# rubychen0611/image-analogies-python

Measured on AMD Instinct MI355X. Metric: B' pixels/sec (brute-force match, 5-level pyramid) + MFMA util @1/2/4/8 GPU, higher is better.
Workload: dtype f16 rotated split (R16 MFMA screen: 3 principal components as f16 pairs, 52 as f16, f32 accumulate) + f64 (rotation, exact rescore, pyramids); 1 GPU; c4: A/A' 2048x2048 x B 1024x1024, 5-level, DB sharded, brute force; levels_cap=5, jobs_per_gpu=1, streams_per_gpu=1, jobs_per_launch=1, parallelism=single

## Files before the change

image-analogies-python_amd/_ia.py:

```python
import ctypes
import os
import re
import sys

import numpy as np
import torch

_HERE = os.path.dirname(os.path.abspath(__file__))
LIB_PATH = os.environ.get('IA_LIB_PATH') or os.path.join(_HERE, 'libia.so')
HEADER = os.path.join(os.path.dirname(_HERE), 'include', 'ia.h')

IA_D = 55
IA_DP = 56

_dp = ctypes.c_void_p


class IaSrcLevel(ctypes.Structure):
    _fields_ = [('A_sm', _dp), ('A_lg', _dp), ('Ap_sm', _dp), ('Ap_lg', _dp),
                ('A_hs', ctypes.c_int), ('A_ws', ctypes.c_int), ('Ah', ctypes.c_int),
                ('Aw', ctypes.c_int), ('nAp', ctypes.c_int)]


class IaLsh(ctypes.Structure):
# ... 141 lines not shown
    'ia_diag_screen3': (ctypes.c_int, [_dp, ctypes.c_long, _dp, ctypes.c_int, _dp, _dp, _dp]),
    'ia_diag_xwave_trace': (ctypes.c_int, [_dp]),
    'ia_diag_set_db_build_form': (ctypes.c_int, [ctypes.c_int]),
    'ia_diag_set_pyr_form': (ctypes.c_int, [ctypes.c_int, ctypes.c_int]),
    'ia_diag_qp_rows': (ctypes.c_int, [ctypes.c_int]),
    'ia_diag_query_rows16': (ctypes.c_int, [_dp, ctypes.c_int, _dp, _dp, _dp, _dp, _dp, _dp]),
    'ia_diag_screen16': (ctypes.c_int, [_dp, ctypes.c_long, _dp, ctypes.c_int, _dp, _dp]),
    'ia_diag_stage_map': (ctypes.c_int, [ctypes.c_long, ctypes.c_long, ctypes.c_int, ctypes.c_int,
                                         ctypes.POINTER(ctypes.c_int)]),
    'ia_diag_screen16_rows': (ctypes.c_int, [ctypes.POINTER(IaSrcLevel), ctypes.c_long, ctypes.c_long,
                                             _dp, _dp, ctypes.c_int, _dp, _dp]),
    'ia_diag_screen16_image': (ctypes.c_int, [ctypes.POINTER(IaSrcLevel), ctypes.c_long,
                                              ctypes.c_long, _dp, _dp, ctypes.c_int, _dp, _dp]),
    'ia_diag_peer_stress': (ctypes.c_int, [_dp, ctypes.c_int, ctypes.c_int,
                                           ctypes.POINTER(ctypes.c_int), _dp]),
    'ia_diag_peer_trace': (ctypes.c_int, [_dp, _dp]),
    'ia_diag_screen16r': (ctypes.c_int, [ctypes.POINTER(IaSrcLevel), ctypes.c_long, ctypes.c_long, _dp, _dp,
                                         _dp, _dp, _dp, ctypes.c_int, _dp, _dp, _dp, _dp, _dp]),
    'ia_diag_screen16k': (ctypes.c_int, [ctypes.POINTER(IaSrcLevel), ctypes.c_long, ctypes.c_long, _dp, _dp,
                                         _dp, _dp, _dp, ctypes.c_int, _dp, _dp, _dp, _dp, _dp]),
    'ia_diag_set_compact_min_rows': (ctypes.c_long, [ctypes.c_long]),
    'ia_diag_wave_compact': (ctypes.c_int, [ctypes.c_int, ctypes.c_int]),
    'ia_diag_compact_waves': (ctypes.c_long, []),
    'ia_diag_wave_rows': (ctypes.c_int, [ctypes.c_int] * 5 + [ctypes.POINTER(ctypes.c_int)]),
    'ia_diag_pipe_schedule': (ctypes.c_int, [ctypes.POINTER(ctypes.c_int)] * 3 + [ctypes.c_int] * 3 +
                              [ctypes.POINTER(ctypes.c_int), ctypes.c_int]),
    'ia_diag_db3_askip': (ctypes.c_int, [_dp, ctypes.c_long, _dp]),
    'ia_diag_screen3r': (ctypes.c_int, [_dp, _dp, _dp, ctypes.c_long, _dp, ctypes.c_int, _dp, _dp, _dp]),
    'ia_diag_synth_level_shards': (ctypes.c_int, [ctypes.POINTER(IaSynthArgs),
                                                  ctypes.POINTER(IaShardDb), ctypes.c_int, _dp]),
}

_lib = None


def declared_symbols(header=None):
    inc = os.path.dirname(HEADER)
    if header == 'all':
        paths = [os.path.join(inc, f) for f in sorted(os.listdir(inc)) if f.endswith('.h')]
    else:
        paths = [header or HEADER]
    names = set()
    for p in paths:
        src = re.sub(r'/\*.*?\*/', '', open(p).read(), flags=re.S)
        names.update(re.findall(r'\b(ia_[a-z0-9_]+)\s*\(', src))
    return sorted(names)
# ... 269 lines not shown
```

image-analogies-python_amd/csrc/ia_internal.h:

```cpp
#pragma once
#include "ia_common.h"

#include <atomic>

namespace ia {

int rot_check_orthonormal(const float *rot, int n, int ld, hipStream_t st, const char *who);
int db_check_amax(const float *amax, hipStream_t st, const char *who);

#ifndef IA_DB_TARGET_CHUNKS
#define IA_DB_TARGET_CHUNKS 512
#endif
constexpr long DB_TARGET_CHUNKS = IA_DB_TARGET_CHUNKS;
extern thread_local long g_db_chunk_target;
constexpr int DB_CHUNK_MAX = 8192;
constexpr int DB_SEG_MAX = 512;

static inline int db_chunk_rows(long nrows) {
    const long target = g_db_chunk_target;
    const long want = (nrows + target * 128 - 1) / (target * 128);
    long tpw = 1;
    while (tpw < want && tpw < DB_CHUNK_MAX / 128) tpw <<= 1;
    return (int)(128 * tpw);
}
// ... 176 lines not shown
    gptr<const float> qp;
    gptr<const double> nq;
    gptr<const float> amax;
    gptr<const double> center;
    gptr<double> q64n;
    gptr<float> qpn;
    gptr<double> nqn;
    gptr<_Float16> q16n;
    ImgPair B, Bp;
    int H, M, y_lo_n, M_n;
    gptr<unsigned long long> dbox;
    gptr<unsigned int> tickets;
    gptr<unsigned int> err;
    gptr<unsigned long long> stats;
    FinishArgs f;
    gptr<const XJob> jobs;
    gptr<unsigned long long> trace;
    gptr<const float> rot;
    gptr<const unsigned char> askc;
    int rk;
    gptr<const unsigned char> restc;
    gptr<const float> rmax;
    gptr<const _Float16> q16;
};
constexpr int XW_TRACE_N = 17, XW_TRACE_PX = 512, XW_TRACE_T = 4096;
constexpr int XW_ROWS = 0, XW_IMG = 1, XW_STRIP = 2;
bool xstrip_applies(const DbSrc &src);
int launch_xwave(const XArgs &a, int nblocks, int form, hipStream_t st, int njobs = 1);

constexpr int STATS_SLOTS = 64, STATS_LINE = 8;
constexpr size_t STATS_BYTES = (size_t)STATS_SLOTS * STATS_LINE * sizeof(unsigned long long);
__device__ __forceinline__ unsigned long long *stats_slot(unsigned long long *s, int q) {
    return s + (q & (STATS_SLOTS - 1)) * STATS_LINE;
}

constexpr size_t MATCH_HEAD = 256;
static inline float *match_segmin(void *scratch) {
    return reinterpret_cast<float *>(reinterpret_cast<char *>(scratch) + MATCH_HEAD);
}
int exact_stage_mode();

int launch_query_wave(const ImgPair &B, const ImgPair &Bp, int t, int y_lo, int M,
                      const double *center, double *q64, float *qp, double *nq,
                      const float *amax, _Float16 *q16, hipStream_t st, const float *rot = nullptr);
int launch_screen16r(const void *dbr, long nrows, const StageMap &sm, const _Float16 *q16, int M,
                     float *segmin, hipStream_t st, const XJob *jobs = nullptr, int njobs = 1, int parity = 0,
                     bool compact = false);
long compact_min_rows();
int launch_db_amax(const IaSrcLevel *src, const DbSrc &d, const double *center, float *amax,
                   double *part, hipStream_t st);
int launch_query_rows(const double *qin, int M, const double *center, float *qp, double *nq,
                      const float *amax, _Float16 *q16, hipStream_t st);
int launch_screen16(const void *db, const ImgDb *img, long nrows, const StageMap &sm,
                    const _Float16 *q16, int M, float *segmin, hipStream_t st,
                    const XJob *jobs = nullptr, int njobs = 1, int parity = 0, bool sharded = false);
size_t match_scratch_bytes(int qrows, long nrows);
int launch_match(const DbSrc &src, long row0, long nrows, const void *db, const void *dbi,
                 const float *qp, const _Float16 *q16, int M, const double *q64, const double *nq,
                 const float *amax, void *scratch, Best *best, unsigned long long *stats,
                 hipStream_t st,
                 hipEvent_t ev0 = nullptr, hipEvent_t ev1 = nullptr,
                 const FinishArgs *fin = nullptr);
int launch_lsh_match(const IaLsh *lsh, const DbSrc &src, long row0, long nrows, int M,
                     const double *q64, const double *center, Best *best,
                     unsigned long long *stats, hipStream_t st);

}
```

image-analogies-python_amd/csrc/ia_synth.hip:

```cpp
#include "ia_finish.h"
#include "ia_split16.h"
#include "ia_rot16.h"
#include "ia_pipe.h"
#include "../../include/ia_diag.h"

#include <cstdio>
#include <cstdlib>
#include <mutex>
#include <vector>

#include <rccl/rccl.h>

namespace ia {

__device__ unsigned int g_sched_err;

__global__ __launch_bounds__(64) void k_err_sticky(const unsigned int *__restrict__ ctl,
                                                   const XJob *__restrict__ jt, int K) {
    for (int k = threadIdx.x; k < K; k += 64) {
        const unsigned int e = jt ? jt[k].ctl[2] : ctl[2];
        if (e) g_sched_err = 1u;
    }
}

// ... 98 lines not shown
    const double d_app = wv == 0 ? app_wdist(src, app, f, qs, lane) : 0.0;
    __syncthreads();
    if (wv == 0) finish_apply(src, app, m, f, cs, d_app, lane);
}

struct SynthWs {
    double *q64;
    float *qp;
    _Float16 *q16;
    double *nq;
    void *scratch;
    Best *best_local;
    ShardRec *rec_local;
    ShardRec *rec_all;
    CohSel *coh;
    unsigned long long *stats;
    double *q64b;
    float *qpb;
    _Float16 *q16b;
    double *nqb;
    unsigned long long *dbox;
    unsigned int *ctl;
    XJob *jtab;
};
constexpr int XW_CTL_ERR = 2;

static size_t carve(SynthWs *ws, char *base, int H, int W, long nrows, int nranks) {
    const int Mmax = wave_max_queries(H, W);
    const int qr = qrows_alloc(Mmax);
    size_t off = 0;
    auto take = [&](size_t bytes) { size_t o = off; off += align_up(bytes, 256); return base ? base + o : nullptr; };
    SynthWs w;
    w.q64 = (double *)take((size_t)Mmax * IA_DP * sizeof(double));
    w.qp = (float *)take((size_t)qr * IA_DP * sizeof(float));
    w.q16 = (_Float16 *)take((size_t)qr * Q16_ROW * 16);
    w.nq = (double *)take((size_t)qr * sizeof(double));
    w.scratch = take(match_scratch_bytes(qr, nrows));
    w.best_local = (Best *)take((size_t)Mmax * sizeof(Best));
    w.rec_local = (ShardRec *)take((size_t)Mmax * sizeof(ShardRec));
    w.rec_all = (ShardRec *)take((size_t)Mmax * nranks * sizeof(ShardRec));
    w.coh = (CohSel *)take((size_t)Mmax * sizeof(CohSel));
    w.stats = (unsigned long long *)take(STATS_BYTES);
    w.q64b = (double *)take((size_t)Mmax * IA_DP * sizeof(double));
    w.qpb = (float *)take((size_t)qr * IA_DP * sizeof(float));
    w.q16b = (_Float16 *)take((size_t)qr * Q16_ROW * 16);
    w.nqb = (double *)take((size_t)qr * sizeof(double));
    w.dbox = (unsigned long long *)take((size_t)H * 2 * sizeof(unsigned long long));
    w.ctl = (unsigned int *)take(256);
    w.jtab = (XJob *)take((size_t)IA_BATCH_MAX * sizeof(XJob));
    if (ws) *ws = w;
    return off;
}

struct GraphKeeper {
    hipStream_t cap = nullptr;
    hipGraphExec_t exec = nullptr;
    hipEvent_t done = nullptr;
    hipError_t retire() {
        if (!exec) return hipSuccess;
        hipError_t e = hipEventSynchronize(done);
        if (e == hipSuccess) e = hipGraphExecDestroy(exec);
        exec = nullptr;
        return e;
    }
    hipError_t hold(hipGraphExec_t x, hipStream_t st) {
        exec = x;
        if (!done) {
            hipError_t e = hipEventCreateWithFlags(&done, hipEventDisableTiming);
            if (e != hipSuccess) return e;
        }
        return hipEventRecord(done, st);
    }
// ... 40 lines not shown
        IA_HIP(hipHostMalloc(&p, STATS_BYTES, hipHostMallocDefault));
        g_prof->pinned.push_back(reinterpret_cast<unsigned long long *>(p));
    }
    *hstats = g_prof->pinned[g_prof->pinned_next++];
    return IA_OK;
}

static hipEvent_t prof_event(size_t i) {
    std::lock_guard<std::mutex> l(g_prof->mu);
    return g_prof->ev[i];
}

static void prof_push(const ProfRec &r) {
    std::lock_guard<std::mutex> l(g_prof->mu);
    g_prof->recs.push_back(r);
}

static std::atomic<int> g_graph_mode{env_int("IA_GRAPH", 0)};
static int graph_mode() { return g_graph_mode.load(std::memory_order_relaxed); }

static std::atomic<long> g_compact_min_rows{1L << 22};
long compact_min_rows() { return g_compact_min_rows.load(std::memory_order_relaxed); }
static std::atomic<long> g_compact_waves{0};

int xwave_attributes(int form, bool rot, hipFuncAttributes *at);
int screen16_attributes(bool img, hipFuncAttributes *at);
int screen_resources_r16(hipFuncAttributes *at);
int comm_allgather(void *comm, const void *send, void *recv, size_t bytes, hipStream_t st);
int comm_nranks(void *comm);
PeerView comm_peer_wave(void *comm);
int comm_peer_mcap(void *comm);

static int shard_tail() {
    static const int v = env_int("IA_SHARD_TAIL", 0);
    return v;
}

static std::atomic<int> g_xwave{env_int("IA_XWAVE", 2)};
static int xwave_on() { return g_xwave.load(std::memory_order_relaxed); }

static unsigned long long *g_xw_trace = nullptr;
static unsigned long long *xw_trace(int tag) {
    static const int want = env_int("IA_XW_TRACE", -1);
    if (want < 0 || tag != want) return nullptr;
    if (!g_xw_trace) {
        const size_t n = (size_t)XW_TRACE_T * XW_TRACE_PX * XW_TRACE_N * sizeof(unsigned long long);
// ... 53 lines not shown
        IA_HIP(hipMemsetAsync(ws.qp, 0, (size_t)qrows_alloc(Mmax) * IA_DP * sizeof(float), st));
        IA_HIP(hipMemsetAsync(ws.q16, 0, (size_t)qrows_alloc(Mmax) * Q16_ROW * 16, st));
        IA_HIP(hipMemsetAsync(ws.stats, 0, STATS_BYTES, st));
        IA_HIP(hipMemsetAsync(ws.scratch, 0, 256, st));
        src = make_dbsrc(a->src);
        B = ImgPair{a->B_sm, a->B_lg, a->B_hs, a->B_ws, H, W};
        Bp = ImgPair{a->Bp_sm, a->Bp_lg, a->B_hs, a->B_ws, H, W};
        prof = !member && (a->flags & IA_SYNTH_PROF) && prof_active();
        timed = prof;
        if (prof && (rc = prof_reserve(3 * (size_t)nw, &ev0, &hstats))) return rc;
        fused = !a->comm && !a->lsh && !sim;
        peer = a->comm && comm_peer_mcap(a->comm) > 0;
        IA_ARG(!peer || comm_peer_mcap(a->comm) >= Mmax,
               "ia_synth_level: the peer exchange's box holds fewer queries than a wave");
        IA_ARG(!peer || a->N_total < (1L << 32),
               "ia_synth_level: the peer exchange carries 32-bit rows (N_total >= 2^32)");
        xw = xwave_on() && !a->lsh && !sim && (!a->comm || peer) && exact_stage_mode() != 1;
        r16 = xw && a->dbr && a->rot;
        IA_HIP(hipMemsetAsync(ws.ctl, 0, 256, st));
        if (xw) {
            IA_HIP(hipMemsetAsync(ws.qpb, 0, (size_t)qrows_alloc(Mmax) * IA_DP * sizeof(float), st));
            IA_HIP(hipMemsetAsync(ws.q16b, 0, (size_t)qrows_alloc(Mmax) * Q16_ROW * 16, st));
            IA_HIP(hipMemsetAsync(ws.dbox, 0, (size_t)H * 2 * sizeof(unsigned long long), st));
        }
        return IA_OK;
    }

    int wave(int t, hipStream_t sq) {
        int y_lo, M;
        wave_rows(H, W, t, y_lo, M);
        if (M <= 0) return IA_OK;
        int rc;
        if (sim) return sim_wave(t, y_lo, M, sq);
        if (xw) return xw_wave(t, y_lo, M, sq);
        if ((rc = launch_query_wave(B, Bp, t, y_lo, M, a->center, ws.q64, ws.qp, ws.nq, a->amax,
                                    ws.q16, sq)))
            return rc;
        hipEvent_t e0 = timed ? prof_event(ev0 + 3 * nscreen) : nullptr;
        hipEvent_t e1 = timed ? prof_event(ev0 + 3 * nscreen + 1) : nullptr;
        FinishArgs fa{t, y_lo, W, a->N_total, a->weights, a->kappa_factor, a->Bp_lg, a->s,
                      a->im, a->dbg_px, a->dbg_dist,
                      a->comm && !peer && shard_tail() ? ws.rec_local : nullptr,
                      a->comm && !peer && shard_tail() ? ws.coh : nullptr};
        if (peer) fa.px = comm_peer_wave(a->comm);
        if (a->lsh) {
            if (e0) IA_HIP(hipEventRecord(e0, sq));
// ... 154 lines not shown
        x.B = B;
        x.Bp = Bp;
        x.H = H; x.M = M; x.y_lo_n = y_lo_n; x.M_n = M_n;
        x.dbox = ws.dbox;
        x.tickets = ws.ctl;
        x.err = ws.ctl + XW_CTL_ERR;
        x.stats = prof ? ws.stats : nullptr;
        x.f = FinishArgs{t, y_lo, W, a->N_total, a->weights, a->kappa_factor, a->Bp_lg, a->s,
                         a->im, a->dbg_px, a->dbg_dist, nullptr, nullptr};
        if (peer) x.f.px = comm_peer_wave(a->comm);
        x.jobs = jt;
        x.trace = xw_trace(a->tag);
        x.rot = r16 ? a->rot : nullptr;
        x.askc = r16 ? r16_askc(a->dbr, a->nrows) : nullptr;
        x.rk = rk ? 1 : 0;
        if (cmp) {
            g_compact_waves.fetch_add(1, std::memory_order_relaxed);
            const char *dbk = reinterpret_cast<const char *>(a->dbk);
            x.restc = reinterpret_cast<const unsigned char *>(dbk + rk_code_off(a->nrows));
            x.rmax = reinterpret_cast<const float *>(dbk + rk_rmax_off(a->nrows));
            x.q16 = q16s[b];
        }
        const int R = M > y_lo_n + M_n - y_lo ? M : y_lo_n + M_n - y_lo;
        if ((rc = launch_xwave(x, R, form, sq, K))) return rc;
        if (timed) IA_HIP(hipEventRecord(prof_event(ev0 + 3 * nscreen + 2), sq));
        ++nscreen;
        pairs += (double)M * (double)a->nrows * K;
        if (prof) Ms.push_back(M);
        static const int sync_every = env_int("IA_SYNC_EVERY", 0);
        if (sync_every > 0 && t % sync_every == sync_every - 1) IA_HIP(hipStreamSynchronize(sq));
        return IA_OK;
    }

    int sim_wave(int t, int y_lo, int M, hipStream_t sq) {
        int rc;
        for (int r = 0; r < nsim; ++r) {
            if ((rc = launch_query_wave(B, Bp, t, y_lo, M, a->center, ws.q64, ws.qp, ws.nq,
                                        sim[r].amax, ws.q16, sq)))
                return rc;
            const FinishArgs fr{t, y_lo, W, a->N_total, a->weights, a->kappa_factor, a->Bp_lg,
                                a->s, a->im, a->dbg_px, a->dbg_dist, ws.rec_all + (long)r * M,
                                ws.coh};
            if ((rc = launch_match(src, sim[r].row0, sim[r].nrows, sim[r].db, sim[r].dbi, ws.qp, ws.q16, M,
                                   ws.q64, ws.nq, sim[r].amax, ws.scratch, ws.best_local, nullptr,
                                   sq, nullptr, nullptr, &fr)))
                return rc;
        }
// ... 127 lines not shown
    if (e) {
        set_error("ia_sched_status: a wait for a neighbouring pixel's decision timed out in some "
                  "level since the last clear (device schedule fault)");
        return IA_E_SCHED;
    }
    return IA_OK;
}

int ia_diag_set_graph_mode(int mode) {
    const int prev = graph_mode();
    if (mode >= 0 && mode <= 2) g_graph_mode.store(mode);
    return prev;
}

int ia_diag_wave_compact(int W, int t) { return wave_compact(W, t) ? 1 : 0; }

long ia_diag_compact_waves(void) { return g_compact_waves.load(std::memory_order_relaxed); }

long ia_diag_set_compact_min_rows(long rows) {
    const long prev = compact_min_rows();
    if (rows >= 0) g_compact_min_rows.store(rows > 0 ? rows : LONG_MAX);
    return prev == LONG_MAX ? 0 : prev;
}

int ia_release_thread_resources(void) {
    IA_HIP(g_graphs.retire());
    IA_HIP(hipDeviceSynchronize());
    {
        const int rc = g_pipe.release();
        if (rc) return rc;
    }
    if (g_graphs.cap) { IA_HIP(hipStreamDestroy(g_graphs.cap)); g_graphs.cap = nullptr; }
    if (g_graphs.done) { IA_HIP(hipEventDestroy(g_graphs.done)); g_graphs.done = nullptr; }
    return IA_OK;
}

int ia_prof_begin(void) {
    std::lock_guard<std::mutex> l(g_prof->mu);
    g_prof->active = true;
    g_prof->next = 0;
    g_prof->pinned_next = 0;
    g_prof->recs.clear();
    return IA_OK;
}

int ia_prof_prepare(long nevents) {
// ... 167 lines not shown
```

image-analogies-python_amd/csrc/ia_xwave.hip:

```cpp
#include "ia_exact.h"
#include "ia_finish.h"
#include "ia_rot16.h"
#include "../../include/ia_diag.h"

#include <climits>

namespace ia {

__device__ __forceinline__ const double *feat_addr(const ImgPair &X, const ImgPair &Y, int r, int c,
                                                   int k, int &rr, int &cc) {
    const bool yk = k >= 34;
    const int kk = yk ? k - 34 : k;
    const bool coarse = kk < 9;
    const int t = coarse ? kk : kk - 9;
    const int xh = coarse ? X.hs : X.h, yh = coarse ? Y.hs : Y.h;
    const int xw = coarse ? X.ws : X.w, yw = coarse ? Y.ws : Y.w;
    const double *xb = coarse ? X.sm : X.lg, *yb = coarse ? Y.sm : Y.lg;
    const int h = yk ? yh : xh;
    const int w = yk ? yw : xw;
    const double *base = yk ? yb : xb;
    const int r0 = coarse ? (r >> 1) + t / 3 - 1 : r + t / 5 - 2;
    const int c0 = coarse ? (c >> 1) + t % 3 - 1 : c + t % 5 - 2;
    rr = symi2(r0, h);
    cc = symi2(c0, w);
// ... 968 lines not shown
            while (mt) {
                const int b = __builtin_ctz(mt);
                mt &= mt - 1;
                if (pos < RESCORE_SEGCAP) slist[pos] = (int)(4 * i + b);
                ++pos;
            }
        }
    }
}
__device__ __forceinline__ void sync3(unsigned *cnt, unsigned g, int lane) {
    asm volatile("s_waitcnt lgkmcnt(0)" ::: "memory");
    if (lane == 0) __hip_atomic_fetch_add(cnt, 1u, __ATOMIC_RELAXED, __HIP_MEMORY_SCOPE_WORKGROUP);
    while (__hip_atomic_load(cnt, __ATOMIC_RELAXED, __HIP_MEMORY_SCOPE_WORKGROUP) < 3u * g)
        __builtin_amdgcn_s_sleep(1);
    asm volatile("" ::: "memory");
}

#ifndef IA_XSTRIP_BOCC
#define IA_XSTRIP_BOCC 4
#endif
#ifndef IA_XSTRIP_BREG
#define IA_XSTRIP_BREG 2
#endif
template <bool BATCH, bool ROT, bool CMP = false>
__global__ __launch_bounds__(256, BATCH ? IA_XSTRIP_BOCC : 3) void k_xstrip(XArgs a0) {
    static_assert(!CMP || (ROT && !BATCH), "compact waves: one job of an R16 level");
    __shared__ __attribute__((aligned(16))) char sa_raw[BATCH ? sizeof(XArgs) : 16];
    XArgs &sa = *reinterpret_cast<XArgs *>(sa_raw);
    if constexpr (BATCH) {
        const unsigned long long *w0 = reinterpret_cast<const unsigned long long *>(&a0);
        unsigned long long *w1 = reinterpret_cast<unsigned long long *>(&sa);
        for (int w = threadIdx.x; w < (int)(sizeof(XArgs) / 8); w += 256) w1[w] = w0[w];
        __syncthreads();
        if (threadIdx.x == 0) xjob_apply(sa, a0.jobs[blockIdx.y], a0.f.t & 1);
        __syncthreads();
    }
    const XArgs &a = BATCH ? sa : a0;
    __shared__ __attribute__((aligned(16))) char win[XS_LDS_B];
    __shared__ double cxd[XW_NCOH * XS_CST];
    __shared__ double cval[XW_NCOH];
    __shared__ double qs[IA_DP], wts[IA_DP];
    __shared__ double cwt[2 * IA_DP];
    __shared__ int slist[RESCORE_SEGCAP];
    __shared__ int tk, scount, sfull;
    __shared__ unsigned bar3;
    __shared__ float redf[4];
    __shared__ double bds[4], bwd[4], bvl[4];
    __shared__ long long bis[4];
    __shared__ CohSel cs;
// ... 2 lines not shown
    __shared__ int cpos[XW_NCOH][3];
    __shared__ unsigned nxw[4][64];
    static_assert(R16_ROT_B + 64 * 8 <= XS_LDS_B, "the rotation fits the window buffer");
    float *const rotl = reinterpret_cast<float *>(win);
    double *const dq = reinterpret_cast<double *>(win + R16_ROT_B);

    const int tid = threadIdx.x, lane = tid & 63, wv = __builtin_amdgcn_readfirstlane(tid >> 6);
    const FinishArgs &f = a.f;
    const DbSrc &src = a.src;
    const int t = f.t, W = f.W;
    const unsigned long long t_start = __builtin_amdgcn_s_memrealtime();
    auto rot_dma = [&]() {
#pragma unroll
        for (int pc = 0; pc < R16_ROT_FLOATS / 256; ++pc)
            __builtin_amdgcn_global_load_lds((const void *)(a.rot.get() + pc * 256 + lane * 4),
                                             (void *)(rotl + pc * 256), 16, 0, 0);
    };
    if (tid == 0) {
        tk = (int)atomicAdd(&a.tickets[t & 1], 1u);
        bar3 = 0;
        scount = 0;
    }
    __syncthreads();
    const int i = tk;
    unsigned long long *trace =
        (a.trace && i < XW_TRACE_PX && t < XW_TRACE_T) ? a.trace + ((long)t * XW_TRACE_PX + i) * XW_TRACE_N : nullptr;
    auto wstamp = [&](int k) {
        if (trace && lane == 0) trace[k] = __builtin_amdgcn_s_memrealtime();
    };
    if (trace && tid == 0) trace[0] = t_start;
    xw_stamp(trace, 1);
    if (i == 0 && tid == 0) __hip_atomic_store(&a.tickets[(t + 1) & 1], 0u, __ATOMIC_RELAXED, __HIP_MEMORY_SCOPE_AGENT);
    const int y = f.y_lo + i, x = t - 3 * y;
    const bool cur = i < a.M;
    const bool nxt = y >= a.y_lo_n && y < a.y_lo_n + a.M_n;

    const float amx = a.amax[vidx(0)];
    int pdep = 0;
    if (wv == 0 && nxt) {
        int rr = 0, cc = 0;
        const double *p = feat_addr_v(a.B.sm, a.B.lg, a.Bp.sm, a.Bp.lg, a.B.h, a.B.w, a.B.hs, a.B.ws, y, x + 1,
                                      lane < IA_D ? lane : 0, rr, cc);
        pdep = lane < 43 || lane >= IA_D ? 0 : (rr == y && cc == x) ? 1 : (rr == y - 1 && cc == x + 3) ? 2 : 0;
        dma_f64(p, lane < IA_D && pdep == 0, nxw[0], nxw[1]);
        dma_f64(a.center + (lane < IA_D ? lane : 0), lane < IA_D, nxw[2], nxw[3]);
    }

    double own = 0.0;
    if (cur) {
        const int t3 = (wv == 0 ? 0 : wv - 1) * 64 + lane;
        const int ql = lane < IA_DP ? lane : 0;
        const double qsv = a.q64[(long)i * IA_DP + ql];
        const double wk0 = f.weights[lane < IA_D ? lane : 0];
        const double wk = lane < IA_D ? wk0 : 0.0;
        const double nqq = a.nq[vidx(i)];
        const double nsk = ROT ? a.q64[(long)i * IA_DP + IA_D] : 0.0;
        const float am = amx, ask = ROT ? a.amax[vidx(1)] : 0.f;
        const long n4 = a.nseg / 4;
        const float4 *sq4 = reinterpret_cast<const float4 *>(a.segmin + (long)i * a.nseg);
        constexpr int XR = BATCH ? IA_XSTRIP_BREG : XS_REG;
        float4 v[XR];
        unsigned sgc[XR];
// ... 17 lines not shown
        const int s_r = f.s[2 * sidx], s_c = f.s[2 * sidx + 1], s_i = f.im[sidx];
        asm volatile("" ::: "memory");
        double Kd = 0.0;
        if constexpr (ROT) Kd = r16_kseg(am, ask, nqq, nsk);
        if (wv != 1) {
            float ewv;
            if constexpr (CMP) {
                const Split16Db sc = split16_db_scale(am);
                const RkKey kq{ldexpf(1.f, sc.ea + split16_q_scale(nqq, sc.R)), (float)sqrt(nrest), rmx / 255.f};
                int ki;
                seg3_wave_seed(sq4, rc4, n4, t3, v, rgc, kq, ewv, ki);
                if (lane == 0) bis[wv] = ki;
            } else if constexpr (ROT) {
                float Kf = (float)Kd;
                if ((double)Kf < Kd) Kf = nextafterf(Kf, INFINITY);
                ewv = seg3_wave_umin(sq4, ac4, n4, t3, v, sgc, Kf);
            } else {
                ewv = seg3_wave_min(sq4, n4, t3, v);
            }
            if (lane == 0) redf[wv] = ewv;
        }
        if (wv == 1) wstamp(14);
        double cv[XW_NCOH], cvl = 0.0;
        if (wv == 1) {
            int sr = s_r + y - rr0, sc = s_c + x - rc0;
            const bool ok = cpos_ok && sr >= 0 && sr < src.A.h && sc >= 0 && sc < src.A.w;
            sr = ok ? sr : 0;
            sc = ok ? sc : 0;
            const int si = ok ? s_i : 0;
            const long cix = ((long)src.A.h * si + sr) * src.A.w + sc;
            cvl = src.Ap.lg[cix];
            if (lane < XW_NCOH) {
                ccix[lane] = ok ? cix : -1;
                cpos[lane][0] = sr; cpos[lane][1] = sc; cpos[lane][2] = si;
            }
            const int k = lane < IA_D ? lane : 0;
            const bool yk = k >= 34;
            const int kk = yk ? k - 34 : k;
            const bool co = kk < 9;
            const int t = co ? kk : kk - 9;
            const int dy = co ? t / 3 - 1 : t / 5 - 2, dx = co ? t % 3 - 1 : t % 5 - 2;
            int Ah = src.A.h, Ahs = src.A.hs, Aw2 = src.A.w, Aws = src.A.ws;
            int hw = (int)src.hw, hws = (int)src.hws;
            const double *pAl = src.A.lg, *pAs = src.A.sm, *pPl = src.Ap.lg, *pPs = src.Ap.sm;
            asm volatile("" : "+v"(Ah), "+v"(Ahs), "+v"(Aw2), "+v"(Aws), "+v"(hw), "+v"(hws));
            asm volatile("" : "+v"(pAl), "+v"(pAs), "+v"(pPl), "+v"(pPs));
            const int ih = co ? Ahs : Ah, iw = co ? Aws : Aw2;
// ... 32 lines not shown
                if (redf[3] < kb || (redf[3] == kb && bis[3] < kl)) { kb = redf[3]; kl = bis[3]; }
                seed = kl >= 0 && kl < a.nseg ? (int)kl : 0;
                xw_stamp(trace, 2);
            }
        } else if (wv != 1) {
            sync3(&bar3, 1, lane);
            const float emin = fminf(redf[0], fminf(redf[2], redf[3]));
            xw_stamp(trace, 2);
            double Tseg, Trow;
            bool force_full;
            if constexpr (ROT) {
                r16_tseg0(emin, am, nqq, Tseg, force_full);
                seg3_select_codes(sq4, ac4, n4, t3, v, sgc, Tseg, Kd, slist, &scount);
            } else {
                rescore_thresholds(emin, am, nqq, Tseg, Trow, force_full);
                seg3_select(sq4, n4, t3, v, Tseg, slist, &scount);
            }
            sync3(&bar3, 2, lane);
            xw_stamp(trace, 3);
            ns = scount;
            full = ns > RESCORE_SEGCAP || force_full;
            if (tid == 0) sfull = full ? 1 : 0;
            if (trace && tid == 0) trace[XW_TRACE_N - 1] = (unsigned long long)(full ? a.nseg : ns);
        }

        auto coherence = [&]() {
#pragma unroll
            for (int c = 0; c < XW_NCOH; ++c) cxd[c * XS_CST + lane] = cv[c];
            if (lane < XW_NCOH) cval[lane] = cvl;
            wave_lds_sync();
            const int c = (lane & 31) < XW_NCOH ? (lane & 31) : XW_NCOH - 1;
            const bool wl = lane >= 32;
            int co = c * XS_CST, qo = 0, wo = wl ? IA_DP : 0;
            asm volatile("" : "+v"(co), "+v"(qo), "+v"(wo));
            Pw55 pw;
#pragma unroll
            for (int k = 0; k < IA_D; ++k) {
                const double xx = (cxd[co + k] - qs[qo + k]) * cwt[wo + k];
                pw.feed(k, xx * xx);
                if (k % 11 == 10) asm volatile("" : "+v"(co), "+v"(qo), "+v"(wo) : "v"(xx));
            }
            const double r = sqrt(pw.res);
            asm volatile("" :: "v"(r));
            const bool valid = (lane & 31) < XW_NCOH && ccix[c] >= 0;
            double bd = valid && !wl ? r : INFINITY;
            long long bl = valid && !wl ? c : LLONG_MAX;
// ... 2 lines not shown
                const double od = __shfl_xor(bd, o);
                const long long ol = __shfl_xor(bl, o);
                fin_best(bd, bl, od, ol);
            }
            const int wn = bl == LLONG_MAX ? 0 : (int)bl;
            const double wd = __shfl(cwd, 32 + wn);
            const double wval = cval[wn];
            wstamp(15);
            if (lane == 0) {
                cs = bl == LLONG_MAX ? CohSel{0, 0, 0, 0, 0, 0, 0, 0.0}
                                     : CohSel{ccix[wn], cpos[wn][0], cpos[wn][1], cpos[wn][2],
                                              y - 2 + wn / 5, x - 2 + wn % 5, 1, wd};
                csval = wval;
            }
        };

        double bd = INFINITY;
        long long bi = LLONG_MAX;
        const int Aw = src.A.w;
        XsWin w{};
        XsFix fx;
        const int dr = wv == 0 ? 0 : wv - 1;
        long nit = CMP ? 0 : full ? a.nseg : ns;
        if (wv != 1 && (CMP || nit > 0)) {
            w = xs_window(a, CMP ? seed : full ? 0 : slist[0]);
            xs_dma(w, src.A, win, dr, lane, fx);
        }
        if (wv == 1) {
            coherence();
        } else if (CMP || nit > 0) {
            win_dma_wait();
            xs_fix(fx, win, 64 * dr + lane);
        }
        if (CMP && tid == 0) bis[1] = seed;
        __syncthreads();
        if (wv == 1) {
            if constexpr (CMP) {
                seed = (int)bis[1];
                w = xs_window(a, seed);
            } else {
                ns = scount;
                full = sfull != 0;
                nit = full ? a.nseg : ns;
                if (nit > 0) w = xs_window(a, full ? 0 : slist[0]);
            }
        }
        long nscan = nit;
        XsPre pre;
        XsWin wn{};
        auto rescore_rows = [&]() {
            const double *wdb = reinterpret_cast<const double *>(win);
            if (w.nst == 4) {
                const int px = w.x0 + (tid & 127), py = w.y0 + 2 * (tid >> 7);
                double d0, d1;
                xs_dist_pair(wdb, xs_fbase(w, py, px), xs_cbase(w, py, px), qs, d0, d1);
                const long g = w.g0 + (long)(2 * (tid >> 7)) * Aw + (tid & 127);
                fin_best(bd, bi, d0, g);
                fin_best(bd, bi, d1, g + Aw);
            } else {
                const int k0 = tid & (a.seg_rows - 1), k1 = (tid + 256) & (a.seg_rows - 1);
                const int y0 = w.y0 + (k0 >> 7), x0 = w.x0 + (k0 & 127);
                const int y1 = w.y0 + (k1 >> 7), x1 = w.x0 + (k1 & 127);
                double d0, d1;
                xs_dist2(wdb, xs_fbase(w, y0, x0), xs_cbase(w, y0, x0), xs_fbase(w, y1, x1), xs_cbase(w, y1, x1),
                         qs, d0, d1);
                if (tid < a.seg_rows) fin_best(bd, bi, d0, w.g0 + (long)(k0 >> 7) * Aw + (k0 & 127));
                if (tid + 256 < a.seg_rows) fin_best(bd, bi, d1, w.g0 + (long)(k1 >> 7) * Aw + (k1 & 127));
            }
// ... 3 lines not shown
            if (wv == 0) wstamp(11);
            rescore_rows();
            if (wv == 0) wstamp(12);
            double um = bd;
            for (int o = 32; o > 0; o >>= 1) um = fmin(um, __shfl_xor(um, o));
            if (lane == 0) bds[wv] = um;
            if (wv != 1) {
                seg3_load(sq4, n4, t3, v);
                seg3_load_codes(ac4, n4, t3, sgc);
                seg3_load_codes(rc4, n4, t3, rgc);
            }
            __syncthreads();
            const double U = fmin(fmin(bds[0], bds[1]), fmin(bds[2], bds[3]));
            bool force_full;
            const RkSel sel = rk_select(U, am, ask, rmx, nqq, nsk, nrest, force_full);
            if (wv != 1) seg3_select_rk(sq4, ac4, rc4, n4, t3, v, sgc, rgc, sel, seed, slist, &scount);
            __syncthreads();
            xw_stamp(trace, 3);
            ns = scount;
            full = ns > RESCORE_SEGCAP || force_full;
            nit = full ? a.nseg : ns;
            nscan = nit + 1;
            if (trace && tid == 0) trace[XW_TRACE_N - 1] = (unsigned long long)nscan;
            if (nit > 0) {
                wn = xs_window(a, full ? 0 : slist[0]);
                xs_pre_load(wn, src.A, tid, pre);
            }
        }
        for (long si = 0; si < nit; ++si) {
            if (si > 0 || CMP) {
                __syncthreads();
                xs_pre_store(pre, win, tid);
                w = wn;
                __syncthreads();
            }
            if (si + 1 < nit) {
                wn = xs_window(a, full ? si + 1 : slist[si + 1]);
                xs_pre_load(wn, src.A, tid, pre);
            }
            if (!CMP && si == 0) {
                xw_stamp(trace, 4);
                if (wv == 0) wstamp(11);
            }
            rescore_rows();
            if (!CMP && si == 0 && wv == 0) wstamp(12);
        }
        for (int o = 32; o > 0; o >>= 1) {
            const double od = __shfl_xor(bd, o);
            const long long oi = __shfl_xor(bi, o);
            fin_best(bd, bi, od, oi);
        }
        XRec wb{bd, bi, 0.0, 0.0};
        if (bi != LLONG_MAX) {
            const long rel = bi - w.g0;
            const long ry = rel >= 0 ? rel / Aw : -1, rx = rel - ry * Aw;
            double sq = 0.0;
            if (rel >= 0 && ry < w.nst && rx < 128) {
                const int py = w.y0 + (int)ry, px = w.x0 + (int)rx;
                const int fb = xs_fbase(w, py, px), cb = xs_cbase(w, py, px);
                const double *wdb = reinterpret_cast<const double *>(win);
                if (lane < IA_D) {
                    const double xw = (wdb[(xs_coarse(lane) ? cb : fb) + xs_koff(lane)] - qs[lane]) * wts[lane];
                    sq = xw * xw;
                }
                wb.val = wdb[XS_FP + fb];
            } else {
                ImgPair ap;
                int r, c;
                src.locate(bi, ap, r, c);
                int rr, cc;
                const double *fp = feat_addr(src.A, ap, r, c, lane < IA_D ? lane : 0, rr, cc);
                if (lane < IA_D) {
                    const double xw = (*fp - qs[lane]) * wts[lane];
                    sq = xw * xw;
                }
                wb.val = src.Ap.lg[bi];
            }
            const double sw = sqrt(pw55_lanes(sq));
            wb.wd = sw * sw;
        }
        if (lane == 0) { bds[wv] = wb.d; bis[wv] = wb.i; bwd[wv] = wb.wd; bvl[wv] = wb.val; }
        __syncthreads();
        xw_stamp(trace, 5);
        if (wv != 0) return;
        if constexpr (ROT) {
            if (nxt) rot_dma();
        }
        XRec lb{INFINITY, LLONG_MAX, 0.0, 0.0};
#pragma unroll
        for (int k = 0; k < 4; ++k) xrec_take(lb, XRec{bds[k], bis[k], bwd[k], bvl[k]});
        xw_stamp(trace, 6);
        own = xw_finish(a, i, y, x, lane, lb, cs, csval, (unsigned int)(nscan * a.seg_rows), ns, full, trace);
    }
    xw_stamp(trace, 8);
    if (wv != 0 || !nxt) return;
    if constexpr (ROT) {
        if (!cur) rot_dma();
    }
    xw_next_query(a, i, y, x, lane, pdep, own, amx, nxw, trace, ROT ? rotl : nullptr, ROT ? dq : nullptr);
}

}

extern "C" int ia_fused_resources(int rot, int *lds, int *vgprs) {
    IA_ARG(lds && vgprs, "ia_fused_resources: bad args");
    hipFuncAttributes at{};
    if (rot) IA_HIP(hipFuncGetAttributes(&at, reinterpret_cast<const void *>(&ia::k_xstrip<false, true>)));
    else IA_HIP(hipFuncGetAttributes(&at, reinterpret_cast<const void *>(&ia::k_xstrip<false, false>)));
    *lds = (int)at.sharedSizeBytes;
    *vgprs = at.numRegs;
    return IA_OK;
}

namespace ia {

int xwave_attributes(int form, bool rot, hipFuncAttributes *at) {
    const void *f = form == XW_STRIP ? (rot ? reinterpret_cast<const void *>(&k_xstrip<false, true>)
                                            : reinterpret_cast<const void *>(&k_xstrip<false, false>))
                    : form == XW_IMG ? reinterpret_cast<const void *>(&k_xwave<true, false>)
                                     : reinterpret_cast<const void *>(&k_xwave<false, false>);
    IA_HIP(hipFuncGetAttributes(at, f));
    return IA_OK;
}

int launch_xwave(const XArgs &a, int nblocks, int form, hipStream_t st, int njobs) {
    if (nblocks <= 0) return IA_OK;
    IA_ARG(njobs >= 1 && njobs <= IA_BATCH_MAX && (njobs == 1 || a.jobs), "launch_xwave: bad batch");
    IA_ARG(form != XW_STRIP || (a.smap.W > 0 && xstrip_applies(a.src) && a.seg_rows >= 128 && a.seg_rows <= 512),
           "launch_xwave: the strip form needs a strip-order image-form level");
    const dim3 grid((unsigned)nblocks, (unsigned)njobs);
    const bool b = njobs > 1;
    IA_ARG(!a.restc || (RK_BUILT && form == XW_STRIP && a.rot && !b && a.rmax && a.q16),
           "launch_xwave: a compact wave is one job of an R16 strip level");
    if (form == XW_STRIP) {
        if (a.restc) {
            k_xstrip<false, true, true><<<grid, 256, 0, st>>>(a);
        } else if (a.rot) {
            if (b) k_xstrip<true, true><<<grid, 256, 0, st>>>(a);
            else k_xstrip<false, true><<<grid, 256, 0, st>>>(a);
        } else {
            if (b) k_xstrip<true, false><<<grid, 256, 0, st>>>(a);
            else k_xstrip<false, false><<<grid, 256, 0, st>>>(a);
        }
    } else if (form == XW_IMG) {
        if (b) k_xwave<true, true><<<grid, 256, 0, st>>>(a);
        else k_xwave<true, false><<<grid, 256, 0, st>>>(a);
    } else {
        if (b) k_xwave<false, true><<<grid, 256, 0, st>>>(a);
        else k_xwave<false, false><<<grid, 256, 0, st>>>(a);
    }
    IA_LAUNCH_CHECK("k_xwave");
    return IA_OK;
}

}
```

include/ia_diag.h:

```cpp
#ifndef IA_DIAG_H
#define IA_DIAG_H

#include <stddef.h>

#include "ia.h"

#ifdef __cplusplus
extern "C" {
#endif

int ia_diag_qp_rows(int M);
int ia_diag_query_rows16(const double *q64, int M, const double *center, const float *amax,
                         float *qp, void *q16, double *nq, void *stream);
int ia_diag_screen16(const void *db, long nrows, const void *q16, int M, float *segmin,
                     void *stream);
int ia_diag_stage_map(long row0, long nrows, int W, int Himg, int *out);
int ia_diag_screen16_rows(const IaSrcLevel *src, long row0, long nrows, const void *db,
                          const void *q16, int M, float *segmin, void *stream);
int ia_diag_screen16_image(const IaSrcLevel *src, long row0, long nrows, const void *dbi,
                           const void *q16, int M, float *segmin, void *stream);
int ia_diag_screen16r(const IaSrcLevel *src, long row0, long nrows, const void *dbr, const float *rot,
                      const float *amax, const double *center, const double *q64, int M, void *q16,
                      double *nq, double *nsk, float *segmin, void *stream);
int ia_diag_screen16k(const IaSrcLevel *src, long row0, long nrows, const void *dbk, const float *rot,
                      const float *amax, const double *center, const double *q64, int M, void *q16,
                      double *nq, double *nsk, float *segmin, void *stream);
long ia_diag_set_compact_min_rows(long rows);
int ia_diag_wave_compact(int W, int t);
long ia_diag_compact_waves(void);
int ia_diag_set_rescore_mode(int mode);
int ia_diag_set_db_build_form(int tiled);
int ia_diag_set_pyr_form(int stream, int oh);
int ia_diag_set_graph_mode(int mode);
int ia_diag_set_xwave(int on);
int ia_diag_set_screen_sched(int sched);
int ia_diag_set_screen_pc(int on);
int ia_diag_set_r16_form(int form);
int ia_diag_set_img_fused(int on);
int ia_diag_screen_trace(void *buf);

int ia_diag_set_color16(int on);
int ia_diag_color16_stats(unsigned long long *out);
int ia_diag_screen3(const void *db3, long nrows, const double *q165, int M, double *e, double *eps,
                    double *qn);
int ia_diag_xwave_trace(unsigned long long *out);

typedef struct {
    const void *db;
    long row0, nrows;
    const float *amax;
    const void *dbi;
} IaShardDb;
// ... 19 lines not shown
```

Before: 2.068 million B' pixels/s.

## Split exact-rescore candidate segments between paired workgroups per query pixel

```diff
diff --git a/image-analogies-python_amd/_ia.py b/image-analogies-python_amd/_ia.py
--- a/image-analogies-python_amd/_ia.py
+++ b/image-analogies-python_amd/_ia.py
@@ -187,6 +187,9 @@
     'ia_diag_set_compact_min_rows': (ctypes.c_long, [ctypes.c_long]),
     'ia_diag_wave_compact': (ctypes.c_int, [ctypes.c_int, ctypes.c_int]),
     'ia_diag_compact_waves': (ctypes.c_long, []),
+    'ia_diag_set_xsplit_min_rows': (ctypes.c_long, [ctypes.c_long]),
+    'ia_diag_xsplit_grid': (ctypes.c_int, [ctypes.c_int, ctypes.c_long, ctypes.c_int]),
+    'ia_diag_xsplit_counts': (ctypes.c_int, [ctypes.POINTER(ctypes.c_ulonglong)]),
     'ia_diag_wave_rows': (ctypes.c_int, [ctypes.c_int] * 5 + [ctypes.POINTER(ctypes.c_int)]),
     'ia_diag_pipe_schedule': (ctypes.c_int, [ctypes.POINTER(ctypes.c_int)] * 3 + [ctypes.c_int] * 3 +
                               [ctypes.POINTER(ctypes.c_int), ctypes.c_int]),
diff --git a/image-analogies-python_amd/csrc/ia_internal.h b/image-analogies-python_amd/csrc/ia_internal.h
--- a/image-analogies-python_amd/csrc/ia_internal.h
+++ b/image-analogies-python_amd/csrc/ia_internal.h
@@ -222,6 +222,7 @@
     gptr<const unsigned char> restc;
     gptr<const float> rmax;
     gptr<const _Float16> q16;
+    gptr<unsigned long long> xbox;
 };
 constexpr int XW_TRACE_N = 17, XW_TRACE_PX = 512, XW_TRACE_T = 4096;
 constexpr int XW_ROWS = 0, XW_IMG = 1, XW_STRIP = 2;
@@ -247,6 +248,7 @@
                      float *segmin, hipStream_t st, const XJob *jobs = nullptr, int njobs = 1, int parity = 0,
                      bool compact = false);
 long compact_min_rows();
+long xsplit_min_rows();
 int launch_db_amax(const IaSrcLevel *src, const DbSrc &d, const double *center, float *amax,
                    double *part, hipStream_t st);
 int launch_query_rows(const double *qin, int M, const double *center, float *qp, double *nq,
diff --git a/image-analogies-python_amd/csrc/ia_synth.hip b/image-analogies-python_amd/csrc/ia_synth.hip
--- a/image-analogies-python_amd/csrc/ia_synth.hip
+++ b/image-analogies-python_amd/csrc/ia_synth.hip
@@ -144,6 +144,7 @@
     unsigned long long *dbox;
     unsigned int *ctl;
     XJob *jtab;
+    unsigned long long *xbox;
 };
 constexpr int XW_CTL_ERR = 2;
 
@@ -170,6 +171,7 @@
     w.dbox = (unsigned long long *)take((size_t)H * 2 * sizeof(unsigned long long));
     w.ctl = (unsigned int *)take(256);
     w.jtab = (XJob *)take((size_t)IA_BATCH_MAX * sizeof(XJob));
+    w.xbox = (unsigned long long *)take((size_t)H * 8 * sizeof(unsigned long long));
     if (ws) *ws = w;
     return off;
 }
@@ -256,6 +258,15 @@
 static std::atomic<long> g_compact_min_rows{1L << 22};
 long compact_min_rows() { return g_compact_min_rows.load(std::memory_order_relaxed); }
 static std::atomic<long> g_compact_waves{0};
+static long xsplit_initial() {
+    const int v = env_int("IA_XSPLIT_MIN_ROWS", 1 << 22);
+    return v > 0 ? v : LONG_MAX;
+}
+static std::atomic<long> g_xsplit_min_rows{xsplit_initial()};
+long xsplit_min_rows() { return g_xsplit_min_rows.load(std::memory_order_relaxed); }
+static int xsplit_grid(bool eligible, long nrows, int R) {
+    return eligible && nrows >= xsplit_min_rows() && db_nsegs(nrows) <= (1L << 20) ? 2 * R : R;
+}
 
 int xwave_attributes(int form, bool rot, hipFuncAttributes *at);
 int screen16_attributes(bool img, hipFuncAttributes *at);
@@ -355,6 +366,7 @@
             IA_HIP(hipMemsetAsync(ws.qpb, 0, (size_t)qrows_alloc(Mmax) * IA_DP * sizeof(float), st));
             IA_HIP(hipMemsetAsync(ws.q16b, 0, (size_t)qrows_alloc(Mmax) * Q16_ROW * 16, st));
             IA_HIP(hipMemsetAsync(ws.dbox, 0, (size_t)H * 2 * sizeof(unsigned long long), st));
+            IA_HIP(hipMemsetAsync(ws.xbox, 0, (size_t)H * 8 * sizeof(unsigned long long), st));
         }
         return IA_OK;
     }
@@ -555,7 +567,9 @@
             x.q16 = q16s[b];
         }
         const int R = M > y_lo_n + M_n - y_lo ? M : y_lo_n + M_n - y_lo;
-        if ((rc = launch_xwave(x, R, form, sq, K))) return rc;
+        const int nwg = xsplit_grid(r16 && K == 1 && !a->comm && form == XW_STRIP, a->nrows, R);
+        if (nwg != R) x.xbox = ws.xbox;
+        if ((rc = launch_xwave(x, nwg, form, sq, K))) return rc;
         if (timed) IA_HIP(hipEventRecord(prof_event(ev0 + 3 * nscreen + 2), sq));
         ++nscreen;
         pairs += (double)M * (double)a->nrows * K;
@@ -729,6 +743,14 @@
     if (rows >= 0) g_compact_min_rows.store(rows > 0 ? rows : LONG_MAX);
     return prev == LONG_MAX ? 0 : prev;
 }
+
+long ia_diag_set_xsplit_min_rows(long rows) {
+    const long prev = xsplit_min_rows();
+    if (rows >= 0) g_xsplit_min_rows.store(rows > 0 ? rows : LONG_MAX);
+    return prev == LONG_MAX ? 0 : prev;
+}
+
+int ia_diag_xsplit_grid(int eligible, long nrows, int R) { return xsplit_grid(eligible != 0, nrows, R); }
 
 int ia_release_thread_resources(void) {
     IA_HIP(g_graphs.retire());
diff --git a/image-analogies-python_amd/csrc/ia_xwave.hip b/image-analogies-python_amd/csrc/ia_xwave.hip
--- a/image-analogies-python_amd/csrc/ia_xwave.hip
+++ b/image-analogies-python_amd/csrc/ia_xwave.hip
@@ -1014,9 +1014,26 @@
 #ifndef IA_XSTRIP_BREG
 #define IA_XSTRIP_BREG 2
 #endif
-template <bool BATCH, bool ROT, bool CMP = false>
+constexpr int XS_RANK_SH = 20;
+constexpr int XS_SEG_MASK = (1 << XS_RANK_SH) - 1;
+__device__ unsigned long long g_xsplit_cnt[2];
+constexpr int XS_SHARE_MIN = 2;
+__device__ __forceinline__ bool xs_helpers(int rank) { return rank & 1; }
+
+__device__ __forceinline__ void xs_rank(int *slist, int ns, int t, int nt) {
+    for (int k = t; k < ns; k += nt) {
+        const int s = __hip_atomic_load(&slist[k], __ATOMIC_RELAXED, __HIP_MEMORY_SCOPE_WORKGROUP) & XS_SEG_MASK;
+        int r = 0;
+        for (int j = 0; j < ns; ++j)
+            r += (__hip_atomic_load(&slist[j], __ATOMIC_RELAXED, __HIP_MEMORY_SCOPE_WORKGROUP) & XS_SEG_MASK) < s ? 1 : 0;
+        __hip_atomic_store(&slist[k], s | (r << XS_RANK_SH), __ATOMIC_RELAXED, __HIP_MEMORY_SCOPE_WORKGROUP);
+    }
+}
+
+template <bool BATCH, bool ROT, bool CMP = false, bool SPLIT = false>
 __global__ __launch_bounds__(256, BATCH ? IA_XSTRIP_BOCC : 3) void k_xstrip(XArgs a0) {
     static_assert(!CMP || (ROT && !BATCH), "compact waves: one job of an R16 level");
+    static_assert(!SPLIT || (ROT && !BATCH), "split candidates: one job of an R16 level");
     __shared__ __attribute__((aligned(16))) char sa_raw[BATCH ? sizeof(XArgs) : 16];
     XArgs &sa = *reinterpret_cast<XArgs *>(sa_raw);
     if constexpr (BATCH) {
@@ -1065,22 +1082,25 @@
         scount = 0;
     }
     __syncthreads();
-    const int i = tk;
+    const int tau = tk;
+    const int i = SPLIT ? tau >> 1 : tau;
+    const bool helper = SPLIT && !(tau & 1);
     unsigned long long *trace =
-        (a.trace && i < XW_TRACE_PX && t < XW_TRACE_T) ? a.trace + ((long)t * XW_TRACE_PX + i) * XW_TRACE_N : nullptr;
+        (!helper && a.trace && i < XW_TRACE_PX && t < XW_TRACE_T) ? a.trace + ((long)t * XW_TRACE_PX + i) * XW_TRACE_N : nullptr;
     auto wstamp = [&](int k) {
         if (trace && lane == 0) trace[k] = __builtin_amdgcn_s_memrealtime();
     };
     if (trace && tid == 0) trace[0] = t_start;
     xw_stamp(trace, 1);
-    if (i == 0 && tid == 0) __hip_atomic_store(&a.tickets[(t + 1) & 1], 0u, __ATOMIC_RELAXED, __HIP_MEMORY_SCOPE_AGENT);
+    if (tau == 0 && tid == 0) __hip_atomic_store(&a.tickets[(t + 1) & 1], 0u, __ATOMIC_RELAXED, __HIP_MEMORY_SCOPE_AGENT);
     const int y = f.y_lo + i, x = t - 3 * y;
     const bool cur = i < a.M;
     const bool nxt = y >= a.y_lo_n && y < a.y_lo_n + a.M_n;
+    if (helper && !cur) return;
 
     const float amx = a.amax[vidx(0)];
     int pdep = 0;
-    if (wv == 0 && nxt) {
+    if (wv == 0 && nxt && !helper) {
         int rr = 0, cc = 0;
         const double *p = feat_addr_v(a.B.sm, a.B.lg, a.Bp.sm, a.Bp.lg, a.B.h, a.B.w, a.B.hs, a.B.ws, y, x + 1,
                                       lane < IA_D ? lane : 0, rr, cc);
@@ -1144,7 +1164,7 @@
         }
         if (wv == 1) wstamp(14);
         double cv[XW_NCOH], cvl = 0.0;
-        if (wv == 1) {
+        if (wv == 1 && !helper) {
             int sr = s_r + y - rr0, sc = s_c + x - rc0;
             const bool ok = cpos_ok && sr >= 0 && sr < src.A.h && sc >= 0 && sc < src.A.w;
             sr = ok ? sr : 0;
@@ -1223,6 +1243,12 @@
             full = ns > RESCORE_SEGCAP || force_full;
             if (tid == 0) sfull = full ? 1 : 0;
             if (trace && tid == 0) trace[XW_TRACE_N - 1] = (unsigned long long)(full ? a.nseg : ns);
+            if constexpr (SPLIT) {
+                if (!full && ns >= XS_SHARE_MIN) {
+                    xs_rank(slist, ns, t3, 192);
+                    sync3(&bar3, 3, lane);
+                }
+            }
         }
 
         auto coherence = [&]() {
@@ -1271,13 +1297,26 @@
         XsFix fx;
         const int dr = wv == 0 ? 0 : wv - 1;
         long nit = CMP ? 0 : full ? a.nseg : ns;
-        if (wv != 1 && (CMP || nit > 0)) {
-            w = xs_window(a, CMP ? seed : full ? 0 : slist[0]);
+        auto mine_from = [&](long k) {
+            if constexpr (SPLIT) {
+                if (!full)
+                    while (k < nit && xs_helpers(slist[k] >> XS_RANK_SH) != helper) ++k;
+            }
+            return k;
+        };
+        auto seg_of = [&](long k) -> long {
+            if constexpr (SPLIT) return full ? k : (long)(slist[k] & XS_SEG_MASK);
+            else return full ? k : (long)slist[k];
+        };
+        if (helper && full) nit = 0;
+        long si0 = CMP ? 0 : mine_from(0);
+        if (wv != 1 && (CMP || si0 < nit)) {
+            w = xs_window(a, CMP ? seed : seg_of(si0));
             xs_dma(w, src.A, win, dr, lane, fx);
         }
         if (wv == 1) {
-            coherence();
-        } else if (CMP || nit > 0) {
+            if (!helper) coherence();
+        } else if (CMP || si0 < nit) {
             win_dma_wait();
             xs_fix(fx, win, 64 * dr + lane);
         }
@@ -1291,8 +1330,13 @@
                 ns = scount;
                 full = sfull != 0;
                 nit = full ? a.nseg : ns;
-                if (nit > 0) w = xs_window(a, full ? 0 : slist[0]);
-            }
+                if (helper && full) nit = 0;
+                si0 = mine_from(0);
+                if (si0 < nit) w = xs_window(a, seg_of(si0));
+            }
+        }
+        if constexpr (SPLIT && !CMP) {
+            if (helper && (full || ns < XS_SHARE_MIN)) return;
         }
         long nscan = nit;
         XsPre pre;
@@ -1342,28 +1386,39 @@
             nit = full ? a.nseg : ns;
             nscan = nit + 1;
             if (trace && tid == 0) trace[XW_TRACE_N - 1] = (unsigned long long)nscan;
-            if (nit > 0) {
-                wn = xs_window(a, full ? 0 : slist[0]);
+            if constexpr (SPLIT) {
+                if (helper && (full || ns < XS_SHARE_MIN)) return;
+                if (!full && ns >= XS_SHARE_MIN) {
+                    xs_rank(slist, ns, tid, 256);
+                    __syncthreads();
+                }
+            }
+            si0 = mine_from(0);
+            if (si0 < nit) {
+                wn = xs_window(a, seg_of(si0));
                 xs_pre_load(wn, src.A, tid, pre);
             }
         }
-        for (long si = 0; si < nit; ++si) {
-            if (si > 0 || CMP) {
+        for (long si = si0; si < nit;) {
+            const bool first = si == si0;
+            const long sn = mine_from(si + 1);
+            if (!first || CMP) {
                 __syncthreads();
                 xs_pre_store(pre, win, tid);
                 w = wn;
                 __syncthreads();
             }
-            if (si + 1 < nit) {
-                wn = xs_window(a, full ? si + 1 : slist[si + 1]);
+            if (sn < nit) {
+                wn = xs_window(a, seg_of(sn));
                 xs_pre_load(wn, src.A, tid, pre);
             }
-            if (!CMP && si == 0) {
+            if (!CMP && first) {
                 xw_stamp(trace, 4);
                 if (wv == 0) wstamp(11);
             }
             rescore_rows();
-            if (!CMP && si == 0 && wv == 0) wstamp(12);
+            if (!CMP && first && wv == 0) wstamp(12);
+            si = sn;
         }
         for (int o = 32; o > 0; o >>= 1) {
             const double od = __shfl_xor(bd, o);
@@ -1404,11 +1459,52 @@
         xw_stamp(trace, 5);
         if (wv != 0) return;
         if constexpr (ROT) {
-            if (nxt) rot_dma();
+            if (nxt && !helper) rot_dma();
         }
         XRec lb{INFINITY, LLONG_MAX, 0.0, 0.0};
 #pragma unroll
         for (int k = 0; k < 4; ++k) xrec_take(lb, XRec{bds[k], bis[k], bwd[k], bvl[k]});
+        if constexpr (SPLIT) {
+            unsigned long long *xb = a.xbox + 8 * (long)y + (lane & 7);
+            if (helper) {
+                const unsigned long long q = (lane & 6) == 0 ? (unsigned long long)__double_as_longlong(lb.d)
+                                           : (lane & 6) == 2 ? (unsigned long long)lb.i
+                                           : (lane & 6) == 4 ? (unsigned long long)__double_as_longlong(lb.wd)
+                                                             : (unsigned long long)__double_as_longlong(lb.val);
+                if (lane < 8)
+                    __hip_atomic_store(xb, dgran(t + 1, (unsigned int)(lane & 1 ? q >> 32 : q)), __ATOMIC_RELAXED,
+                                       __HIP_MEMORY_SCOPE_AGENT);
+                if (lane == 0) atomicAdd(&g_xsplit_cnt[0], 1ULL);
+                return;
+            }
+            if (!full && ns >= XS_SHARE_MIN) {
+                unsigned long long g = 0;
+                bool dead = false;
+                const unsigned long long t0 = __builtin_amdgcn_s_memrealtime();
+                for (;;) {
+                    g = __hip_atomic_load(xb, __ATOMIC_RELAXED, __HIP_MEMORY_SCOPE_AGENT);
+                    if (__all((unsigned)(g >> 32) == (unsigned)(t + 1))) break;
+                    if (__builtin_amdgcn_s_memrealtime() - t0 > PEER_TIMEOUT_TICKS) {
+                        if (lane == 0) atomicOr(a.err, 1u);
+                        dead = true;
+                        break;
+                    }
+                    __builtin_amdgcn_s_sleep(1);
+                }
+                if (a.stats && lane == 0)
+                    atomicAdd(&stats_slot(a.stats, i)[4], __builtin_amdgcn_s_memrealtime() - t0);
+                if (!dead) {
+                    auto word = [&](int k) {
+                        return ((unsigned long long)(unsigned)__shfl((int)(unsigned)g, k + 1) << 32) |
+                               (unsigned)__shfl((int)(unsigned)g, k);
+                    };
+                    const XRec hr{__longlong_as_double((long long)word(0)), (long long)word(2),
+                                  __longlong_as_double((long long)word(4)), __longlong_as_double((long long)word(6))};
+                    if (lane == 0 && (hr.d < lb.d || (hr.d == lb.d && hr.i < lb.i))) atomicAdd(&g_xsplit_cnt[1], 1ULL);
+                    xrec_take(lb, hr);
+                }
+            }
+        }
         xw_stamp(trace, 6);
         own = xw_finish(a, i, y, x, lane, lb, cs, csval, (unsigned int)(nscan * a.seg_rows), ns, full, trace);
     }
@@ -1429,6 +1525,14 @@
     else IA_HIP(hipFuncGetAttributes(&at, reinterpret_cast<const void *>(&ia::k_xstrip<false, false>)));
     *lds = (int)at.sharedSizeBytes;
     *vgprs = at.numRegs;
+    return IA_OK;
+}
+
+extern "C" int ia_diag_xsplit_counts(unsigned long long *out) {
+    IA_ARG(out, "ia_diag_xsplit_counts: bad args");
+    IA_HIP(hipDeviceSynchronize());
+    IA_HIP(hipMemcpyFromSymbol(out, HIP_SYMBOL(ia::g_xsplit_cnt), 2 * sizeof(unsigned long long), 0,
+                               hipMemcpyDeviceToHost));
     return IA_OK;
 }
 
@@ -1452,8 +1556,13 @@
     const bool b = njobs > 1;
     IA_ARG(!a.restc || (RK_BUILT && form == XW_STRIP && a.rot && !b && a.rmax && a.q16),
            "launch_xwave: a compact wave is one job of an R16 strip level");
+    IA_ARG(!a.xbox || (form == XW_STRIP && a.rot && !b && !a.f.px.nranks && a.nseg <= XS_SEG_MASK + 1),
+           "launch_xwave: split candidates are for one unsharded job of an R16 strip level");
     if (form == XW_STRIP) {
-        if (a.restc) {
+        if (a.xbox) {
+            if (a.restc) k_xstrip<false, true, true, true><<<grid, 256, 0, st>>>(a);
+            else k_xstrip<false, true, false, true><<<grid, 256, 0, st>>>(a);
+        } else if (a.restc) {
             k_xstrip<false, true, true><<<grid, 256, 0, st>>>(a);
         } else if (a.rot) {
             if (b) k_xstrip<true, true><<<grid, 256, 0, st>>>(a);
diff --git a/include/ia_diag.h b/include/ia_diag.h
--- a/include/ia_diag.h
+++ b/include/ia_diag.h
@@ -28,6 +28,9 @@
 long ia_diag_set_compact_min_rows(long rows);
 int ia_diag_wave_compact(int W, int t);
 long ia_diag_compact_waves(void);
+long ia_diag_set_xsplit_min_rows(long rows);
+int ia_diag_xsplit_grid(int eligible, long nrows, int R);
+int ia_diag_xsplit_counts(unsigned long long *out);
 int ia_diag_set_rescore_mode(int mode);
 int ia_diag_set_db_build_form(int tiled);
 int ia_diag_set_pyr_form(int stream, int oh);
```

Result: faster. 2.093 million B' pixels/s, median of 6 (+1.2%).
